# NuTufts/ubresnet

Hardware: AMD Instinct MI355X
Metric: images/sec, 512x512 U-ResNet train step (fwd+loss+bwd+Adam) (higher is better)
Workload: dtype bf16; 1 GPU; ub_uresnet 3-class ip16 bf16, batch 16 per GPU (global 16), 512x512x1 synthetic LArTPC crops, Adam(1e-5, wd 1e-4); parallelism=dp1, global_batch=16, optimizer=ubresnet_amd.optim.FlatAdam

## Files before the change

### ubresnet_amd/csrc/ubr_conv.hip

```cpp
#include <stdlib.h>
#include <type_traits>
#include "ubr_common.h"
#include "ubr_host.h"

namespace {

struct ConvK {
  const char* x; long x_sn, x_sy, x_sx;
  const float *in_sub, *in_scale, *in_shift, *in_lo;
  const char* w;
  char* y; long y_sn, y_sy, y_sx;
  const char* ad; long a_sn, a_sy, a_sx;
  const float* bias;
  double* stats;
  int H, W;
  int CU, UPB, lgUPB, nblk;
  int Cout, Cout_pad;
  int ntaps, S, iy0, ix0, OH, OW;
  int dymin, dxmin, HH, HW;
  int tiles_x, tiles_y;
  unsigned tx_magic, ty_magic;
  int nunits, steps;
  int pixb;
  unsigned rw, rw_magic;
// ... 531 lines not shown
        }
        const int vo = (okp[i] && okc[j]) ? lane_y : kOut;
        if constexpr (sizeof(T) == 2) {
          uint2 pk;
          store4<T>(reinterpret_cast<char*>(&pk), v);
          __builtin_amdgcn_raw_buffer_store_b64(ubr_u2{pk.x, pk.y}, yr, vo, so_y[i] + j * 16 * ESZ, 0);
        } else {
          buf_store16(ubr_u4{__float_as_uint(v[0]), __float_as_uint(v[1]), __float_as_uint(v[2]), __float_as_uint(v[3])}, yr, vo, so_y[i] + j * 16 * ESZ);
        }
      }
    }
  } else
#pragma unroll
  for (int j = 0; j < NT; ++j) {
    const int ch = n0 + j * 16 + 4 * q;
    float4 bmu = make_float4(0.f, 0.f, 0.f, 0.f), bsc = bmu, bsh = bmu, bis = bmu;
    const bool bnb = k.bc != nullptr && ch < k.Cout;
    if (bnb) {
      bmu = *reinterpret_cast<const float4*>(k.bmean + ch); bsc = *reinterpret_cast<const float4*>(k.bscale + ch);
      bsh = *reinterpret_cast<const float4*>(k.bshift + ch); bis = *reinterpret_cast<const float4*>(k.binvstd + ch);
    }
    auto finish = [&](int i, float* v, int& oy, int& ox) -> bool {
      const int f = wave * FW + i;
      oy = oy0 + f / TWF; ox = ox0 + (f % TWF) * 16 + l16;
      const bool valid = (oy < k.OH) && (ox < k.OW);
#pragma unroll
      for (int r = 0; r < 4; ++r) v[r] = acc[i][j][r] + bs[j][r];
      if (k.act & 1) {
#pragma unroll
        for (int r = 0; r < 4; ++r) v[r] = fmaxf(v[r], 0.f);
      }
      if (adb != nullptr && valid && ch < k.Cout) {
        float a4[4];
        load4<T>(adb + (long)n * k.a_sn + (long)oy * k.a_sy + (long)ox * k.a_sx + (long)ch * ESZ, a4);
        if (k.ad_mask != nullptr) {
          const unsigned mb = (unsigned)k.ad_mask[(((long)n * k.OH + oy) * k.OW + ox) * k.ad_mask_cu + ch / CPU] >> (ch % CPU);
#pragma unroll
          for (int r = 0; r < 4; ++r) a4[r] = ((mb >> r) & 1u) ? a4[r] : 0.f;
        }
#pragma unroll
        for (int r = 0; r < 4; ++r) v[r] += a4[r];
      }
      if (k.act & 2) {
#pragma unroll
        for (int r = 0; r < 4; ++r) v[r] = fmaxf(v[r], 0.f);
      }
      if (k.stats != nullptr && valid) {
        if (k.bc != nullptr) {
          if (bnb) {
            float g4[4], c4[4];
            round4<T>(v, g4);
            load4<T>(k.bc + (long)n * k.bc_sn + (long)oy * k.bc_sy + (long)ox * k.bc_sx + (long)ch * ESZ, c4);
            bnb_accumulate(g4, c4, bmu, bsc, bsh, bis, s1[j], s2[j]);
          }
        } else {
#pragma unroll
          for (int r = 0; r < 4; ++r) { s1[j][r] += v[r]; s2[j][r] += v[r] * v[r]; }
        }
      }
      return valid;
    };
    constexpr bool PAIRS = (FW % 2 == 0) && sizeof(T) == 2;
    if (PAIRS && k.pair_store && k.epilogue == 0) {
#pragma unroll
      for (int i = 0; i < FW; i += 2) {
        float v0[4], v1[4];
        int oy_a, ox_a, oy_b, ox_b;
        const bool ok0 = finish(i, v0, oy_a, ox_a) && ch < k.Cout;
        const bool ok1 = finish(i + (FW > 1 ? 1 : 0), v1, oy_b, ox_b) && ch < k.Cout;
        store_frag_pair<T>(yb + (long)n * k.y_sn + (long)oy_a * k.y_sy + (long)ox_a * k.y_sx + (long)ch * ESZ,
                           yb + (long)n * k.y_sn + (long)oy_b * k.y_sy + (long)ox_b * k.y_sx + (long)ch * ESZ, ok0, ok1, v0, v1, q);
      }
    } else {
#pragma unroll
    for (int i = 0; i < FW; ++i) {
      float v[4];
      int oy, ox;
      const bool valid = finish(i, v, oy, ox);
      if (k.epilogue == 0) {
        if (valid && ch < k.Cout)
          store4<T>(yb + (long)n * k.y_sn + (long)oy * k.y_sy + (long)ox * k.y_sx + (long)ch * ESZ, v);
      } else if (j == 0) {
        float m = -3.0e38f;
#pragma unroll
        for (int r = 0; r < 4; ++r) if (ch + r < k.Cout) m = fmaxf(m, v[r]);
        m = fmaxf(m, __shfl_xor(m, 16, 64));
        m = fmaxf(m, __shfl_xor(m, 32, 64));
        float e = 0.f;
#pragma unroll
        for (int r = 0; r < 4; ++r) if (ch + r < k.Cout) e += expf(v[r] - m);
        e += __shfl_xor(e, 16, 64);
        e += __shfl_xor(e, 32, 64);
        const float lse = m + logf(e);
        if (valid) {
          float* o = reinterpret_cast<float*>(k.y);
#pragma unroll
          for (int r = 0; r < 4; ++r)
            if (ch + r < k.Cout) o[(((long)n * k.Cout + ch + r) * k.OH + oy) * k.OW + ox] = v[r] - lse;
        }
      }
    }
    }
  }

#ifdef UBR_CONV_STAMPS
  const unsigned long long te1 = __builtin_amdgcn_s_memtime();
#endif
  if (k.stats != nullptr) {
#pragma unroll
    for (int j = 0; j < NT; ++j)
#pragma unroll
      for (int r = 0; r < 4; ++r) {
        const float a = wave_quadrow_sum16(s1[j][r]);
        const float b = wave_quadrow_sum16(s2[j][r]);
        if (l16 == 0) {
          red[(wave * TN + j * 16 + 4 * q + r) * 2 + 0] = a;
          red[(wave * TN + j * 16 + 4 * q + r) * 2 + 1] = b;
        }
      }
    __syncthreads();
    if (tid < TN) {
      const int ch = n0 + tid;
      if (ch < k.Cout) {
        double a = 0.0, b = 0.0;
#pragma unroll
        for (int w = 0; w < 4; ++w) { a += (double)red[(w * TN + tid) * 2]; b += (double)red[(w * TN + tid) * 2 + 1]; }
        double* st = k.stats + (size_t)(blockIdx.x % k.nslots) * 2 * k.Cout;
        atomicAdd(&st[ch], a);
        atomicAdd(&st[k.Cout + ch], b);
      }
    }
  }
#ifdef UBR_CONV_STAMPS
  if (PIPE && k.stamps != nullptr) {
    const unsigned long long te2 = __builtin_amdgcn_s_memtime();
    __syncthreads();
    if (tid == 0) {
      unsigned long long* o = k.stamps + ((size_t)blockIdx.y * gridDim.x + blockIdx.x) * 16;
      o[9] = __builtin_amdgcn_s_memtime(); o[11] = te0; o[12] = te1; o[13] = te2;
    }
  }
#endif
}

struct ThinK {
  const char* x; long x_sn; int x_sy, x_sx; unsigned x_bytes;
  const float *in_sub, *in_scale, *in_shift, *in_lo;
  const char* w;
  char* y; long y_sn; int y_sy, y_sx; unsigned y_bytes;
  const char* ad; long a_sn; int a_sy, a_sx; unsigned a_bytes;
  const float* bias; double* stats;
  int H, W, HW, nitems; unsigned hw_magic;
  int tiles_x, tiles_y, ntiles; unsigned tx_magic, ty_magic;
  int steps, nunits, hy_org, hx_org, dymin, dxmin;
  int Cout, Cout_pad, CU, OH, OW;
  int act, epilogue, wlinear, dbg;
  int wl_off, halo_off, red_off;
  int8_t dy[UBR_MAX_TAPS], dx[UBR_MAX_TAPS];
  uint8_t wt[UBR_MAX_TAPS];
  unsigned long long* stamps;
  const uint8_t* ad_mask; int ad_mask_cu; unsigned mask_bytes;
  const char* bc; long bc_sn; int bc_sy, bc_sx; unsigned bc_bytes;
  const float *bmean, *bscale, *bshift, *binvstd;
  int nslots;
  int nphase, pstep0[4], psteps[4], pyoff[4];
};


template <typename T, int FW, int NT, int TWF, int UPB, bool XF, bool LSM, bool ROW7 = false, int EXT = 0>
__global__ __launch_bounds__(256, ((ROW7 || (EXT == 1 && NT == 2)) ? 2 : 3)) void conv_thin_kernel(const ThinK k) {
  ubr_main_prio();
  static_assert(EXT == 0 || (!XF && !LSM), "the training epilogues belong to the data-gradient convs (no transform on load, NHWC output)");
  constexpr int TN = NT * 16;
  constexpr int TH = 4 * FW / TWF;
  constexpr int TW = TWF * 16;
  constexpr int CPU = ET<T>::CPU;
  constexpr int ESZ = 16 / CPU;
  constexpr int LG = UPB == 4 ? 2 : (UPB == 2 ? 1 : 0);
  constexpr int PIXB = thin_pixb(UPB);
  constexpr int HS = ROW7 ? 7 : (UPB == 4 ? 6 : 5);
  constexpr int PPS = 256 / UPB;
  constexpr int WB = 4;
  constexpr int FH = ROW7 ? 8 : 4;
  static_assert(TWF == 2 && FW % FH == 0, "tile shape");
  static_assert(!ROW7 || (FW == 8 && NT == 1 && UPB == 2), "ROW7 is the 16x32-pixel, 16-cout, 16-cin tile");
  constexpr bool WIDE = ESZ == 2;

  extern __shared__ __attribute__((aligned(16))) char smem[];
  int* tbl = reinterpret_cast<int*>(smem);
  char* wl = smem + k.wl_off;
  char* halo = smem + k.halo_off;
  float* red = reinterpret_cast<float*>(smem + k.red_off);

  const int tid = threadIdx.x, lane = tid & 63, wave = tid >> 6, q = lane >> 4, l16 = lane & 15;
  const int n0 = blockIdx.y * TN;
  const int c = tid & (UPB - 1);
  const int nw = 4 * k.steps * TN;

  int hxu[HS], relu[HS];
  int hyu[XF ? HS : 1];
#pragma unroll
  for (int u = 0; u < HS; ++u) {
    const int pix = (tid >> LG) + u * PPS;
    const int hy = (int)udiv_magic((unsigned)pix, k.hw_magic), hx = pix - hy * k.HW;
    const bool in = tid + u * 256 < k.nitems;
    hxu[u] = in ? hx : -(1 << 24);
    relu[u] = hy * k.x_sy + hx * k.x_sx + c * 16;
    if constexpr (XF) hyu[u] = hy;
  }
  char* const halo_w = halo + (tid >> LG) * PIXB + c * 16;

  ubr_u4 hv[HS];
  unsigned hok = 0u;
  auto load_halo = [&](int tile) {
    const unsigned t = (unsigned)__builtin_amdgcn_readfirstlane(tile);
    const unsigned r = udiv_magic(t, k.tx_magic), tx = t - r * (unsigned)k.tiles_x;
    const unsigned n = udiv_magic(r, k.ty_magic), ty = r - n * (unsigned)k.tiles_y;
    const int hy0 = (int)ty * TH + k.hy_org, hx0 = (int)tx * TW + k.hx_org;
    __amdgpu_buffer_rsrc_t xr = __builtin_amdgcn_make_buffer_rsrc((void*)(k.x + (long)n * k.x_sn), 0, (int)k.x_bytes, 0x00020000);
    const int goff = hy0 * k.x_sy + hx0 * k.x_sx;
    hok = 0u;
#pragma unroll
    for (int u = 0; u < HS; ++u) {
      const bool ok = (unsigned)(hx0 + hxu[u]) < (unsigned)k.W;
      int vo = ok ? relu[u] + goff : -1;
      if (k.dbg & 1) vo = -1;
      hv[u] = __builtin_amdgcn_raw_buffer_load_b128(xr, vo, 0, 0);
      if constexpr (XF) hok |= (unsigned)(ok & ((unsigned)(hy0 + hyu[u]) < (unsigned)k.H)) << u;
    }
  };

  const int ntiles = k.ntiles;
  int tile = blockIdx.x;
  load_halo(tile);
  uint4 wv[WB];
  if (k.wlinear) {
    const int nvalid = k.nunits * TN;
#pragma unroll
    for (int u = 0; u < WB; ++u) {
      const int i = tid + u * 256;
      wv[u] = make_uint4(0u, 0u, 0u, 0u);
      if (i < nvalid) wv[u] = ldg16(k.w + (long)i * 16);
    }
  }
  float bs[NT][4];
#pragma unroll
  for (int j = 0; j < NT; ++j)
#pragma unroll
    for (int r = 0; r < 4; ++r) {
      const int ch = n0 + j * 16 + 4 * q + r;
      bs[j][r] = (k.bias != nullptr && ch < k.Cout) ? k.bias[ch] : 0.f;
    }
  float* xfc = red + 4 * TN * 2;
  if constexpr (XF) {
    for (int i = tid; i < 4 * UPB * CPU; i += 256) {
      const int which = i / (UPB * CPU), ch = i - which * (UPB * CPU);
      const float* src = which == 0 ? k.in_sub : (which == 1 ? k.in_scale : (which == 2 ? k.in_shift : k.in_lo));
      xfc[i] = src[ch];
    }
  }
  if constexpr (EXT == 1) {
    for (int i = tid; i < 4 * TN; i += 256) {
      const int which = i / TN, ch = n0 + (i - which * TN);
      const float* src = which == 0 ? k.bmean : (which == 1 ? k.bscale : (which == 2 ? k.bshift : k.binvstd));
      xfc[i] = ch < k.Cout ? src[ch] : 0.f;
    }
  }
  int* wsrc = tbl + 4 * k.steps;
  for (int u = tid; u < 4 * k.steps; u += 256) {
    int off = 0, v = -1;
    if (u < k.nunits) {
      const int tap = u >> LG, cc = u & (UPB - 1);
      off = ((k.dy[tap] - k.dymin) * k.HW + (k.dx[tap] - k.dxmin)) * PIXB + cc * 16;
      v = k.wt[tap] == 255 ? -1 : ((int)k.wt[tap] * k.CU + cc) * k.Cout_pad;
    }
    tbl[u] = off;
    wsrc[u] = v;
  }
  if (k.wlinear) {
#pragma unroll
    for (int u = 0; u < WB; ++u) {
      const int i = tid + u * 256;
      if (i < nw) *reinterpret_cast<uint4*>(wl + (long)i * 16) = wv[u];
    }
    const int nvalid = k.nunits * TN;
    for (int ib = tid + 256 * WB; ib < nw; ib += 256 * WB) {
#pragma unroll
      for (int u = 0; u < WB; ++u) {
        const int i = ib + u * 256;
        wv[u] = make_uint4(0u, 0u, 0u, 0u);
        if (i < nvalid) wv[u] = ldg16(k.w + (long)i * 16);
      }
#pragma unroll
      for (int u = 0; u < WB; ++u) {
        const int i = ib + u * 256;
        if (i < nw) *reinterpret_cast<uint4*>(wl + (long)i * 16) = wv[u];
      }
    }
  } else {
    __syncthreads();
    for (int ib = tid; ib < nw; ib += 256 * WB) {
#pragma unroll
      for (int u = 0; u < WB; ++u) {
        const int i = ib + u * 256;
        wv[u] = make_uint4(0u, 0u, 0u, 0u);
        if (i < nw) {
          const int src = wsrc[i / TN];
          if (src >= 0) wv[u] = ldg16(k.w + ((long)(src + n0 + (i % TN))) * 16);
        }
      }
#pragma unroll
      for (int u = 0; u < WB; ++u) {
        const int i = ib + u * 256;
        if (i < nw) *reinterpret_cast<uint4*>(wl + (long)i * 16) = wv[u];
      }
    }
  }

  if constexpr (XF || EXT == 1) __syncthreads();
  const int fb0 = (((wave * FW) / TWF) * k.HW + l16) * PIXB;
  const int rowb = k.HW * PIXB;
  int vo_out[NT];
#pragma unroll
  for (int j = 0; j < NT; ++j) {
    if constexpr (WIDE) vo_out[j] = ((wave * FW) / TWF) * k.y_sy + ((q & 1) * 16 + l16) * k.y_sx + (n0 + j * 16 + 8 * (q >> 1)) * ESZ;
    else vo_out[j] = ((wave * FW) / TWF) * k.y_sy + l16 * k.y_sx + (n0 + j * 16 + 4 * q) * ESZ;
  }
  int vo_ad[NT];
#pragma unroll
  for (int j = 0; j < NT; ++j) vo_ad[j] = ((wave * FW) / TWF) * k.a_sy + l16 * k.a_sx + (n0 + j * 16 + 4 * q) * ESZ;
  int vo_c[EXT == 1 ? NT : 1], vo_m[EXT == 2 ? NT : 1];
  if constexpr (EXT == 1) {
#pragma unroll
    for (int j = 0; j < NT; ++j) vo_c[j] = ((wave * FW) / TWF) * k.bc_sy + l16 * k.bc_sx + (n0 + j * 16 + 4 * q) * ESZ;
  }
  if constexpr (EXT == 2) {
#pragma unroll
    for (int j = 0; j < NT; ++j) vo_m[j] = (((wave * FW) / TWF) * k.OW + l16) * k.ad_mask_cu + (n0 + j * 16 + 4 * q) / CPU;
  }
  float s1[NT][4], s2[NT][4];
#pragma unroll
  for (int j = 0; j < NT; ++j)
#pragma unroll
    for (int r = 0; r < 4; ++r) { s1[j][r] = 0.f; s2[j][r] = 0.f; }

#ifdef UBR_CONV_STAMPS
  unsigned long long tS = 0, tL = 0, tC = 0, tE = 0, tB = 0, tW = 0, t_ = __builtin_amdgcn_s_memtime();
  const unsigned long long t_begin = t_;
#define UBR_TSTAMP(acc_) do { unsigned long long n_ = __builtin_amdgcn_s_memtime(); acc_ += n_ - t_; t_ = n_; } while (0)
#else
#define UBR_TSTAMP(acc_) do { } while (0)
#endif
  while (tile < ntiles) {
#ifdef UBR_CONV_STAMPS
    asm volatile("s_waitcnt vmcnt(0)" ::: "memory");
    UBR_TSTAMP(tW);
#endif
    float xsub[XF ? CPU : 1], xsc[XF ? CPU : 1], xsh[XF ? CPU : 1], xlo[XF ? CPU : 1];
    if constexpr (XF) {
#pragma unroll
      for (int e = 0; e < CPU; ++e) {
        xsub[e] = xfc[0 * UPB * CPU + c * CPU + e]; xsc[e] = xfc[1 * UPB * CPU + c * CPU + e];
        xsh[e] = xfc[2 * UPB * CPU + c * CPU + e]; xlo[e] = xfc[3 * UPB * CPU + c * CPU + e];
      }
    }
#pragma unroll
    for (int u = 0; u < HS; ++u) {
      uint4 v = __builtin_bit_cast(uint4, hv[u]);
      if constexpr (XF) {
        if ((hok >> u) & 1u) {
          float f[CPU];
          ET<T>::unpack(v, f);
          ubr_bnrelu<CPU>(f, xsub, xsc, xsh, xlo);
          v = ET<T>::pack(f);
        }
      }
      if (tid + u * 256 < k.nitems) *reinterpret_cast<uint4*>(halo_w + u * (PPS * PIXB)) = v;
    }
    UBR_TSTAMP(tS);
    __syncthreads();
    UBR_TSTAMP(tB);
    const unsigned t = (unsigned)__builtin_amdgcn_readfirstlane(tile);
    const unsigned rr = udiv_magic(t, k.tx_magic), tx = t - rr * (unsigned)k.tiles_x;
    const unsigned n = udiv_magic(rr, k.ty_magic), ty = rr - n * (unsigned)k.tiles_y;
    const int oy0 = (int)ty * TH, ox0 = (int)tx * TW;
    const int next = tile + gridDim.x;
    if (next < ntiles) load_halo(next);
    __amdgpu_buffer_rsrc_t yr = __builtin_amdgcn_make_buffer_rsrc((void*)(k.y + (long)n * k.y_sn), 0, (int)k.y_bytes, 0x00020000);
    __amdgpu_buffer_rsrc_t ar = __builtin_amdgcn_make_buffer_rsrc((void*)(k.ad != nullptr ? k.ad + (long)n * k.a_sn : k.x), 0, k.ad != nullptr ? (int)k.a_bytes : 0, 0x00020000);
    const int ybase = oy0 * k.y_sy + ox0 * k.y_sx, abase = oy0 * k.a_sy + ox0 * k.a_sx;
    __amdgpu_buffer_rsrc_t cr = yr, mr = yr;
    int cbase = 0, mbase = 0;
    if constexpr (EXT == 1) {
      cr = __builtin_amdgcn_make_buffer_rsrc((void*)(k.bc + (long)n * k.bc_sn), 0, (int)k.bc_bytes, 0x00020000);
      cbase = oy0 * k.bc_sy + ox0 * k.bc_sx;
    }
    if constexpr (EXT == 2) {
      mr = __builtin_amdgcn_make_buffer_rsrc((void*)(k.ad_mask + (long)n * k.mask_bytes), 0, (int)k.mask_bytes, 0x00020000);
      mbase = (oy0 * k.OW + ox0) * k.ad_mask_cu;
    }
    UBR_TSTAMP(tL);

#pragma unroll 1
    for (int g0 = 0; g0 < FW; g0 += FH) {
      ubr_u4 adv4[FH][NT];
      ubr_u2 adv2[FH][NT];
      if (k.ad != nullptr) {
#pragma unroll
        for (int i = 0; i < FH; ++i)
#pragma unroll
          for (int j = 0; j < NT; ++j) {
            const int so = abase + ((g0 + i) / TWF) * k.a_sy;
            if constexpr (WIDE) adv2[i][j] = __builtin_amdgcn_raw_buffer_load_b64(ar, vo_ad[j] + (i % TWF) * 16 * k.a_sx, so, 0);
            else adv4[i][j] = __builtin_amdgcn_raw_buffer_load_b128(ar, vo_ad[j] + (i % TWF) * 16 * k.a_sx, so, 0);
          }
      }
      unsigned admk[EXT == 2 ? FH : 1][EXT == 2 ? NT : 1];
      ubr_u4 cv4[EXT == 1 ? FH : 1][EXT == 1 ? NT : 1];
      ubr_u2 cv2[EXT == 1 ? FH : 1][EXT == 1 ? NT : 1];
      if constexpr (EXT == 2) {
#pragma unroll
        for (int i = 0; i < FH; ++i)
#pragma unroll
          for (int j = 0; j < NT; ++j)
            admk[i][j] = __builtin_amdgcn_raw_buffer_load_b8(mr, vo_m[j] + (i % TWF) * 16 * k.ad_mask_cu, mbase + ((g0 + i) / TWF) * k.OW * k.ad_mask_cu, 0);
      }
      if constexpr (EXT == 1) {
#pragma unroll
        for (int i = 0; i < FH; ++i)
#pragma unroll
          for (int j = 0; j < NT; ++j) {
            const int so = cbase + ((g0 + i) / TWF) * k.bc_sy;
            if constexpr (WIDE) cv2[i][j] = __builtin_amdgcn_raw_buffer_load_b64(cr, vo_c[j] + (i % TWF) * 16 * k.bc_sx, so, 0);
            else cv4[i][j] = __builtin_amdgcn_raw_buffer_load_b128(cr, vo_c[j] + (i % TWF) * 16 * k.bc_sx, so, 0);
          }
      }
      const int nph = (ROW7 || LSM || EXT != 0) ? 1 : k.nphase;
#pragma unroll 1
      for (int ph = 0; ph < nph; ++ph) {
      const int s_lo = nph > 1 ? k.pstep0[ph] : 0;
      const int s_cnt = nph > 1 ? k.psteps[ph] : k.steps;
      const int y_ph = nph > 1 ? k.pyoff[ph] : 0;
      f32x4 acc[FH][NT];
#pragma unroll
      for (int i = 0; i < FH; ++i)
#pragma unroll
        for (int j = 0; j < NT; ++j) acc[i][j] = f32x4{0.f, 0.f, 0.f, 0.f};
      const char* hb = halo + fb0 + (g0 / TWF) * rowb;
      if constexpr (ROW7) {
        constexpr int ROWB = (TW + 6) * PIXB;
#pragma unroll 1
        for (int pp = 0; pp < 4; ++pp) {
          const char* pb = hb + tbl[4 * pp + q];
          const char* pw = wl + ((4 * pp + q) * TN + l16) * 16;
          uint4 w7[7];
#pragma unroll
          for (int dy = 0; dy < 7; ++dy) w7[dy] = *reinterpret_cast<const uint4*>(pw + dy * (16 * TN * 16));
#pragma unroll
          for (int ir = 0; ir < 10; ++ir) {
            const uint4 b0 = *reinterpret_cast<const uint4*>(pb + ir * ROWB);
            const uint4 b1 = *reinterpret_cast<const uint4*>(pb + ir * ROWB + 16 * PIXB);
#pragma unroll
            for (int r = 0; r < 4; ++r) {
              const int dy = ir - r;
              if (dy >= 0 && dy <= 6) {
                acc[2 * r][0] = mma_step<T>(acc[2 * r][0], w7[dy], b0);
                acc[2 * r + 1][0] = mma_step<T>(acc[2 * r + 1][0], w7[dy], b1);
              }
            }
          }
        }
      } else {
      int off_n = tbl[4 * s_lo + q];
      uint4 wf_n[NT];
#pragma unroll
      for (int j = 0; j < NT; ++j) wf_n[j] = *reinterpret_cast<const uint4*>(wl + (((4 * s_lo + q) * TN) + j * 16 + l16) * 16);
      const int nsteps = s_lo + ((k.dbg & 2) ? 1 : s_cnt);
      for (int s = s_lo; s < nsteps; ++s) {
        const char* pa = hb + off_n;
        uint4 wf[NT];
#pragma unroll
        for (int j = 0; j < NT; ++j) wf[j] = wf_n[j];
        if (s + 1 < nsteps) {
          off_n = tbl[4 * (s + 1) + q];
#pragma unroll
          for (int j = 0; j < NT; ++j) wf_n[j] = *reinterpret_cast<const uint4*>(wl + (((4 * (s + 1) + q) * TN) + j * 16 + l16) * 16);
        }
        uint4 a[FH];
        a[0] = *reinterpret_cast<const uint4*>(pa);
        a[1] = *reinterpret_cast<const uint4*>(pa + 16 * PIXB);
        a[2] = *reinterpret_cast<const uint4*>(pa + rowb);
        a[3] = *reinterpret_cast<const uint4*>(pa + rowb + 16 * PIXB);
#pragma unroll
        for (int i = 0; i < FH; ++i)
#pragma unroll
          for (int j = 0; j < NT; ++j) acc[i][j] = mma_step<T>(acc[i][j], wf[j], a[i]);
      }
      }
      UBR_TSTAMP(tC);

#pragma unroll
      for (int i = 0; i < FH; i += 2) {
#pragma unroll
        for (int j = 0; j < NT; ++j) {
          float v[2][4];
#pragma unroll
          for (int h = 0; h < 2; ++h) {
#pragma unroll
            for (int r = 0; r < 4; ++r) v[h][r] = acc[i + h][j][r] + bs[j][r];
            if (k.act & 1) {
#pragma unroll
              for (int r = 0; r < 4; ++r) v[h][r] = fmaxf(v[h][r], 0.f);
            }
            if (k.ad != nullptr) {
              float a4[4];
              if constexpr (WIDE) {
                const uint2 raw = make_uint2(adv2[i + h][j][0], adv2[i + h][j][1]);
                load4<T>(reinterpret_cast<const char*>(&raw), a4);
              } else {
                const uint4 raw = __builtin_bit_cast(uint4, adv4[i + h][j]);
                ET<T>::unpack(raw, a4);
              }
              if constexpr (EXT == 2) {
                const unsigned mb = (admk[i + h][j] & 0xffu) >> ((n0 + j * 16 + 4 * q) % CPU);
#pragma unroll
                for (int r = 0; r < 4; ++r) v[h][r] = __builtin_fmaf(a4[r], (float)((mb >> r) & 1u), v[h][r]);
              } else {
#pragma unroll
                for (int r = 0; r < 4; ++r) v[h][r] += a4[r];
              }
            }
            if (k.act & 2) {
#pragma unroll
              for (int r = 0; r < 4; ++r) v[h][r] = fmaxf(v[h][r], 0.f);
            }
            if constexpr (EXT == 1) {
              float g4[4], c4[4];
              round4<T>(v[h], g4);
              if constexpr (WIDE) {
                const uint2 raw = make_uint2(cv2[i + h][j][0], cv2[i + h][j][1]);
                load4<T>(reinterpret_cast<const char*>(&raw), c4);
              } else {
                const uint4 raw = __builtin_bit_cast(uint4, cv4[i + h][j]);
                ET<T>::unpack(raw, c4);
              }
              const float* cc = xfc + j * 16 + 4 * q;
              bnb_accumulate(g4, c4, *reinterpret_cast<const float4*>(cc), *reinterpret_cast<const float4*>(cc + TN),
                             *reinterpret_cast<const float4*>(cc + 2 * TN), *reinterpret_cast<const float4*>(cc + 3 * TN), s1[j], s2[j]);
            } else if (k.stats != nullptr) {
#pragma unroll
              for (int r = 0; r < 4; ++r) { s1[j][r] += v[h][r]; s2[j][r] += v[h][r] * v[h][r]; }
            }
          }
          const int so = ybase + ((g0 + i) / TWF) * k.y_sy + y_ph;
          if constexpr (!LSM) {
            if (k.dbg & 4) {
              if (v[0][0] == 1.2345e-30f && v[1][1] == 1.2345e-30f) __builtin_amdgcn_raw_buffer_store_b32(__float_as_uint(v[0][0]), yr, vo_out[j], so, 0);
            } else if constexpr (WIDE) {
              const uint4 pk = pack_swap_pair<T>(v[0], v[1]);
              ubr_u4 o = {pk.x, pk.y, pk.z, pk.w};
              buf_store16(o, yr, vo_out[j], so);
            } else {
#pragma unroll
              for (int h = 0; h < 2; ++h) {
                ubr_u4 o = {__float_as_uint(v[h][0]), __float_as_uint(v[h][1]), __float_as_uint(v[h][2]), __float_as_uint(v[h][3])};
                buf_store16(o, yr, vo_out[j] + h * 16 * k.y_sx, so);
              }
            }
          } else if (j == 0) {
            (void)so;
#pragma unroll
            for (int h = 0; h < 2; ++h) {
              const int ch = 4 * q;
              const int f = wave * FW + g0 + i + h;
              const int oy = oy0 + f / TWF, ox = ox0 + (f % TWF) * 16 + l16;
              float m = -3.0e38f;
#pragma unroll
              for (int r = 0; r < 4; ++r) if (ch + r < k.Cout) m = fmaxf(m, v[h][r]);
              m = fmaxf(m, __shfl_xor(m, 16, 64));
              m = fmaxf(m, __shfl_xor(m, 32, 64));
              float e = 0.f;
#pragma unroll
              for (int r = 0; r < 4; ++r) if (ch + r < k.Cout) e += expf(v[h][r] - m);
              e += __shfl_xor(e, 16, 64);
              e += __shfl_xor(e, 32, 64);
              const float lse = m + logf(e);
              float* o = reinterpret_cast<float*>(k.y);
#pragma unroll
              for (int r = 0; r < 4; ++r)
                if (ch + r < k.Cout) o[(((long)n * k.Cout + ch + r) * k.OH + oy) * k.OW + ox] = v[h][r] - lse;
            }
          }
        }
      }
      }
      UBR_TSTAMP(tE);
    }
    tile = next;
    if (tile < ntiles) __syncthreads();
    UBR_TSTAMP(tB);
  }
#ifdef UBR_CONV_STAMPS
  if (k.stamps != nullptr && tid == 0) {
    unsigned long long* o = k.stamps + ((size_t)blockIdx.y * gridDim.x + blockIdx.x) * 16;
    o[0] = tS; o[1] = tL; o[2] = tC; o[3] = tB; o[6] = tW; o[10] = tE; o[4] = t_ - t_begin; o[5] = t_begin; o[7] = t_begin; o[8] = t_; o[9] = t_;
  }
#endif

  if (k.stats != nullptr) {
#pragma unroll
    for (int j = 0; j < NT; ++j)
#pragma unroll
      for (int r = 0; r < 4; ++r) {
        const float a = wave_quadrow_sum16(s1[j][r]);
        const float b = wave_quadrow_sum16(s2[j][r]);
        if (l16 == 0) {
          red[(wave * TN + j * 16 + 4 * q + r) * 2 + 0] = a;
          red[(wave * TN + j * 16 + 4 * q + r) * 2 + 1] = b;
        }
      }
    __syncthreads();
    if (tid < TN) {
      const int ch = n0 + tid;
      if (ch < k.Cout) {
        double a = 0.0, b = 0.0;
#pragma unroll
        for (int w = 0; w < 4; ++w) { a += (double)red[(w * TN + tid) * 2]; b += (double)red[(w * TN + tid) * 2 + 1]; }
        double* st = k.stats + (size_t)(blockIdx.x % k.nslots) * 2 * k.Cout;
        atomicAdd(&st[ch], a);
        atomicAdd(&st[k.Cout + ch], b);
      }
    }
  }
}

template <typename T, int FW, int TWF, int STEPS>
__global__ __launch_bounds__(512) void conv_pc_kernel(const ConvK k) {
  constexpr int NT = 4, TN = 64;
  constexpr int F = 4 * FW;
  constexpr int TH = F / TWF;
  constexpr int TW = TWF * 16;
  constexpr int CPU = ET<T>::CPU;
  constexpr int ESZ = 16 / CPU;
  constexpr int HS = conv_pipe_hslots(FW, TWF), WS = conv_pipe_wslots(NT);
  constexpr int kOOR = (int)0x80000000;
  static_assert(F % TWF == 0, "tile shape");

  extern __shared__ __attribute__((aligned(16))) char smem[];
  int* tbl = reinterpret_cast<int*>(smem);
  int* wsrc = tbl + 4 * k.steps;
  float* xfc = reinterpret_cast<float*>(smem + k.xfc_off);

  const int tid = threadIdx.x, lane = tid & 63, wave = tid >> 6, q = lane >> 4, l16 = lane & 15;
  const bool producer = wave >= 4;
  const int ptid = tid & 255;
  const bool has_xf = k.in_scale != nullptr;

  for (int u = tid; u < 4 * k.steps; u += 512) {
    int off = 0, v = -1;
    if (u < k.nunits) {
      const int tap = u >> 2, cc = u & 3;
      off = ((k.dy[tap] - k.dymin) * k.HW + (k.dx[tap] - k.dxmin)) * k.pixb + cc * 16;
      v = ((int)k.wt[tap] * k.CU + cc) * k.Cout_pad;
    }
    tbl[u] = off;
    wsrc[u] = v;
  }
  if (has_xf) {
    for (int ch = tid; ch < k.CU * CPU; ch += 512) {
      float* o = xfc + (ch / CPU) * 4 * CPU + (ch % CPU);
      o[0] = k.in_sub[ch]; o[CPU] = k.in_scale[ch]; o[2 * CPU] = k.in_shift[ch]; o[3 * CPU] = k.in_lo[ch];
    }
  }
  __syncthreads();

  const int ntiles = k.tiles_x * k.tiles_y * k.N;
  const int total = ntiles * k.ncot;
  const int G = (int)gridDim.x;
  const int nmine = (int)blockIdx.x < total ? (total - (int)blockIdx.x + G - 1) / G : 0;
  const int niter = nmine * k.nblk;

  float s1[NT][4], s2[NT][4];
#pragma unroll
  for (int j = 0; j < NT; ++j)
#pragma unroll
    for (int r = 0; r < 4; ++r) { s1[j][r] = 0.f; s2[j][r] = 0.f; }

  if (producer) {
    const int c = ptid & 3;
    const int nit = k.HH * (int)k.rw;
    const int nw = 4 * k.steps * TN;
    int h_rc[HS], h_rel[HS];
#pragma unroll
    for (int u = 0; u < HS; ++u) {
      const int it = ptid + u * 256;
      const int hy = (int)__umulhi((unsigned)it, k.rw_magic);
      const int hx = (it - hy * (int)k.rw) >> 2;
      h_rc[u] = it < nit ? ((hy << 16) | hx) : -1;
      h_rel[u] = hy * k.x_sy32 + hx * k.x_sx32 + c * 16;
    }
    int w_rel[WS];
#pragma unroll
    for (int u = 0; u < WS; ++u) {
      const int i = ptid + u * 256;
      int v = kOOR;
      if (i < nw) {
        const int src = wsrc[i / TN];
        if (src >= 0) v = (src + (i % TN)) * 16;
      }
      w_rel[u] = v;
    }
    const __amdgpu_buffer_rsrc_t wr = __builtin_amdgcn_make_buffer_rsrc((void*)k.w, 0, 0x7fffffff, 0x00020000);
    const int x_img = k.H * k.x_sy32;
    const int hfull = nit >> 8, hrem = nit & 255, wfull = nw >> 8, wrem = nw & 255;
    const int halo_inc = 64 * k.pixb;
    char* const halo_w0 = smem + k.halo_off + (ptid >> 2) * k.pixb + c * 16;
    char* const wl_w0 = smem + k.wl_off + ptid * 16;

    int lu = (int)blockIdx.x, lblk = 0;
    int hoff[HS], woff[WS];
    unsigned hok_unit = 0u;
    __amdgpu_buffer_rsrc_t xr = wr;
    auto issue = [&](ubr_u4 (&hv)[HS], ubr_u4 (&wv)[WS], unsigned& hokm) {
      if (lblk == 0) {
        const int u_ = __builtin_amdgcn_readfirstlane(lu);
        const int ct = u_ / ntiles;
        int t = u_ - ct * ntiles;
        const int tx = t % k.tiles_x; t /= k.tiles_x;
        const int ty = t % k.tiles_y;
        const int n = t / k.tiles_y;
        const int hy0 = ty * TH + k.iy0 + k.dymin, hx0 = tx * TW + k.ix0 + k.dxmin;
        xr = __builtin_amdgcn_make_buffer_rsrc((void*)(k.x + (long)n * k.x_sn), 0, x_img, 0x00020000);
        const int org = hy0 * k.x_sy32 + hx0 * k.x_sx32;
        hok_unit = 0u;
#pragma unroll
        for (int u = 0; u < HS; ++u) {
          const int hy = h_rc[u] >> 16, hx = h_rc[u] & 0xffff;
          const bool okx = h_rc[u] >= 0 && (unsigned)(hx0 + hx) < (unsigned)k.W;
          hoff[u] = okx ? h_rel[u] + org : kOOR;
          hok_unit |= (okx && (unsigned)(hy0 + hy) < (unsigned)k.H) ? (1u << u) : 0u;
        }
        const int n0b = ct * TN * 16;
#pragma unroll
        for (int u = 0; u < WS; ++u) woff[u] = w_rel[u] == kOOR ? kOOR : w_rel[u] + n0b;
      }
      const int sh = lblk * 64, sw = lblk * 4 * k.Cout_pad * 16;
#pragma unroll
      for (int u = 0; u < HS; ++u) hv[u] = __builtin_amdgcn_raw_buffer_load_b128(xr, hoff[u], sh, 0);
#pragma unroll
      for (int u = 0; u < WS; ++u) wv[u] = __builtin_amdgcn_raw_buffer_load_b128(wr, woff[u], sw, 0);
      hokm = hok_unit;
      if (++lblk == k.nblk) { lblk = 0; lu += G; }
// ... 329 lines not shown
      unsigned long long* o = k.stamps + (size_t)blockIdx.x * 16;
      o[0] = tC; o[1] = tE; o[2] = tB; o[3] = t_ - t_begin; o[4] = (unsigned long long)niter;
    }
#endif
  }
}

static thread_local int g_last_conv_cfg[4] = {0, 0, 0, 0};
static thread_local char g_last_conv_name[160] = "";
struct TileCfg { int FW, NT, TWF; };
static const TileCfg kCfgs[] = {
    {8, 1, 2},
    {4, 1, 2},
    {4, 2, 2},
    {4, 4, 2},
    {2, 4, 1},
    {1, 4, 1},
    {2, 2, 1},
    {2, 1, 1},
    {1, 2, 1},
    {1, 1, 1},
};
constexpr int kNumCfgs = sizeof(kCfgs) / sizeof(kCfgs[0]);

template <typename T, int FW, int NT, int TWF, bool PIPE>
int launch_one(const ConvK& k, dim3 grid, size_t lds, hipStream_t st) {
  auto fn = conv_igemm_kernel<T, FW, NT, TWF, PIPE>;
  if (lds > 64 * 1024) {
    static thread_local size_t maxset = 0;
    if (lds > maxset) {
      hipError_t e = hipFuncSetAttribute(reinterpret_cast<const void*>(fn), hipFuncAttributeMaxDynamicSharedMemorySize, (int)lds);
      if (e != hipSuccess) { ubr_set_error("ubr_conv: cannot raise LDS limit to %zu: %s", lds, hipGetErrorString(e)); return UBR_ELAUNCH; }
      maxset = lds;
    }
  }
  ubr_launch(fn, grid, dim3(256), lds, st, k);
  UBR_LAUNCH_CHECK("ubr_conv");
  return UBR_OK;
}

template <typename T, int FW, int NT, int TWF, int UPB, bool XF, bool LSM = false, bool ROW7 = false, int EXT = 0>
int launch_thin(const ThinK& k, dim3 grid, size_t lds, hipStream_t st) {
  auto fn = conv_thin_kernel<T, FW, NT, TWF, UPB, XF, LSM, ROW7, EXT>;
  if (lds > 64 * 1024) {
    static thread_local size_t maxset = 0;
    if (lds > maxset) {
      hipError_t e = hipFuncSetAttribute(reinterpret_cast<const void*>(fn), hipFuncAttributeMaxDynamicSharedMemorySize, (int)lds);
      if (e != hipSuccess) { ubr_set_error("ubr_conv: cannot raise LDS limit to %zu: %s", lds, hipGetErrorString(e)); return UBR_ELAUNCH; }
      maxset = lds;
    }
  }
  ubr_launch(fn, grid, dim3(256), lds, st, k);
  UBR_LAUNCH_CHECK("ubr_conv");
  return UBR_OK;
}

static unsigned magic_u32(unsigned d) { return d <= 1 ? 0u : (unsigned)((0x100000000ull + d - 1) / d); }

template <typename T, int FW, int NT, int TWF>
int try_thin(const ConvK& c, dim3 grid, hipStream_t st, int* rc) {
  constexpr int TH = 4 * FW / TWF, TW = TWF * 16, TN = NT * 16;
  static const bool thin_on = [] { const char* e = getenv("UBR_CONV_THIN"); return !e || atoi(e) != 0; }();
  const int esz = 16 / ET<T>::CPU;
  if (!thin_on || c.nblk != 1 || c.S != 1 || (c.UPB != 2 && c.UPB != 4)) return 0;
  const int nph = (int)grid.z;
  int steps_tot = c.steps, nunits_tot = c.nunits;
  if (nph > 1) {
    if (nph > 4 || c.ad != nullptr || c.stats != nullptr || c.epilogue != 0 || c.bc != nullptr || c.ad_mask != nullptr) return 0;
    steps_tot = 0; nunits_tot = 0;
    for (int p = 0; p < nph; ++p) {
      if (c.pnunits[p] % 4 || c.ptap0[p] * c.UPB != nunits_tot || c.pyoff[p] < 0 || c.pyoff[p] >= (1L << 30)) return 0;
      steps_tot += c.psteps[p]; nunits_tot += c.pnunits[p];
    }
    if (nunits_tot != c.ntaps * c.UPB) return 0;
  }
  int map7[7][7];
  bool row7 = false;
  if constexpr (FW == 8 && NT == 1 && sizeof(T) == 2) {
    static const bool row7_on = [] { const char* e = getenv("UBR_CONV_ROW7"); return !e || atoi(e) != 0; }();
    row7 = row7_on && c.ntaps == 49 && c.UPB == 2 && c.dymin == -3 && c.dxmin == -3 && c.HW == TW + 6 && c.HH == TH + 6;
    if (row7) {
      for (int a = 0; a < 7; ++a) for (int b = 0; b < 7; ++b) map7[a][b] = -1;
      for (int t = 0; t < 49 && row7; ++t) {
        const int a = c.dy[t] + 3, b = c.dx[t] + 3;
        if (a < 0 || a > 6 || b < 0 || b > 6 || map7[a][b] >= 0 || c.wt[t] == 255) row7 = false; else map7[a][b] = c.wt[t];
      }
    }
  }
  const int HSn = row7 ? 7 : (c.UPB == 4 ? 6 : 5);
  if (c.HH * (int)c.rw > 256 * HSn) return 0;
  if (c.OH % TH || c.OW % TW) return 0;
  if (c.epilogue == 0 && esz == 2 && !c.wide_store) return 0;
  if (c.epilogue == 0 && (c.Cout % 4 || c.Cout_pad != (int)grid.y * TN)) return 0;
  if (c.x_sy >= (1L << 24) || c.y_sy >= (1L << 24) || (long)c.H * c.x_sy >= (1L << 31) || (long)c.OH * c.y_sy >= (1L << 31)) return 0;
  if (c.ad != nullptr && (c.a_sy >= (1L << 24) || (long)c.OH * c.a_sy >= (1L << 31))) return 0;
  const int ntiles = c.tiles_x * c.tiles_y * c.N;
  if ((unsigned long long)ntiles * (unsigned)c.tiles_x >= (1ull << 32)) return 0;
  ThinK k{};
  k.x = c.x; k.x_sn = c.x_sn; k.x_sy = (int)c.x_sy; k.x_sx = (int)c.x_sx; k.x_bytes = (unsigned)((long)c.H * c.x_sy);
  k.in_sub = c.in_sub; k.in_scale = c.in_scale; k.in_shift = c.in_shift; k.in_lo = c.in_lo;
  k.w = c.w;
  k.y = c.y; k.y_sn = c.y_sn; k.y_sy = (int)c.y_sy; k.y_sx = (int)c.y_sx; k.y_bytes = (unsigned)((long)c.OH * c.y_sy);
  k.ad = c.ad; k.a_sn = c.a_sn; k.a_sy = (int)c.a_sy; k.a_sx = (int)c.a_sx; k.a_bytes = c.ad ? (unsigned)((long)c.OH * c.a_sy) : 0u;
  k.bias = c.bias; k.stats = c.stats;
  k.H = c.H; k.W = c.W; k.HW = c.HW; k.nitems = c.HH * (int)c.rw; k.hw_magic = magic_u32((unsigned)c.HW);
  k.tiles_x = c.tiles_x; k.tiles_y = c.tiles_y; k.ntiles = ntiles;
  k.tx_magic = magic_u32((unsigned)c.tiles_x); k.ty_magic = magic_u32((unsigned)c.tiles_y);
  k.steps = steps_tot; k.nunits = nunits_tot; k.hy_org = c.iy0 + c.dymin; k.hx_org = c.ix0 + c.dxmin; k.dymin = c.dymin; k.dxmin = c.dxmin;
  k.nphase = nph;
  for (int p = 0, s0 = 0; p < 4; ++p) {
    k.pstep0[p] = s0; k.psteps[p] = p < nph ? c.psteps[p] : 0; k.pyoff[p] = p < nph ? (int)c.pyoff[p] : 0;
    s0 += k.psteps[p];
  }
  k.Cout = c.Cout; k.Cout_pad = c.Cout_pad; k.CU = c.CU; k.OH = c.OH; k.OW = c.OW;
  k.act = c.act; k.epilogue = c.epilogue; k.wlinear = nph > 1 ? 0 : c.wlinear; k.dbg = c.dbg; k.stamps = c.stamps;
  for (int t = 0; t < c.ntaps; ++t) { k.dy[t] = c.dy[t]; k.dx[t] = c.dx[t]; k.wt[t] = c.wt[t]; }
  const int ext = c.bc != nullptr ? 1 : (c.ad_mask != nullptr ? 2 : 0);
  if (ext != 0 && (c.in_scale != nullptr || c.epilogue != 0)) return 0;
  k.nslots = c.nslots;
  if (ext == 1) {
    if (c.bc_sy >= (1L << 24) || (long)c.OH * c.bc_sy >= (1L << 31)) return 0;
    k.bc = c.bc; k.bc_sn = c.bc_sn; k.bc_sy = (int)c.bc_sy; k.bc_sx = (int)c.bc_sx; k.bc_bytes = (unsigned)((long)c.OH * c.bc_sy);
    k.bmean = c.bmean; k.bscale = c.bscale; k.bshift = c.bshift; k.binvstd = c.binvstd;
  }
  if (ext == 2) {
    if ((long)c.OH * c.OW * c.ad_mask_cu >= (1L << 31)) return 0;
    k.ad_mask = c.ad_mask; k.ad_mask_cu = c.ad_mask_cu; k.mask_bytes = (unsigned)((long)c.OH * c.OW * c.ad_mask_cu);
  }
  if (row7) {
    for (int a = 0; a < 7; ++a)
      for (int b = 0; b < 8; ++b) {
        const int t = a * 8 + b;
        k.dy[t] = (int8_t)(a - 3); k.dx[t] = (int8_t)((b < 7 ? b : 6) - 3); k.wt[t] = (uint8_t)(b < 7 ? map7[a][b] : 255);
      }
    k.nunits = 56 * 2; k.steps = 28; k.wlinear = 0;
  }
  const int pixb = thin_pixb(c.UPB);
  size_t off = ((size_t)2 * 16 * k.steps + 15) & ~(size_t)15;
  k.wl_off = (int)off; off += (size_t)4 * k.steps * TN * 16;
  k.halo_off = (int)off; off += ((size_t)c.HH * c.HW * pixb + 15) & ~(size_t)15;
  k.red_off = (int)off; off += (size_t)4 * TN * 2 * sizeof(float) + (size_t)4 * 4 * 8 * sizeof(float);
  const size_t lds = off;
  if (lds > 150 * 1024) return 0;
  const size_t lds_budget = 159 * 1024;
  static const int wg_per_cu = [] { const char* e = getenv("UBR_CONV_THIN_WGS"); return e ? atoi(e) : 0; }();
  int per_cu = (int)(lds_budget / lds);
  const int reg_cap = (row7 || (ext == 1 && NT == 2)) ? 2 : (NT == 1 ? (ext == 1 ? 3 : 4) : 3);
  if (per_cu > reg_cap) per_cu = reg_cap;
  if (wg_per_cu > 0) per_cu = wg_per_cu;
  if (per_cu < 1) per_cu = 1;
  dim3 g(grid.x, grid.y);
  const unsigned cap = 256u * (unsigned)per_cu / (grid.y ? grid.y : 1);
  if (g.x > cap && cap > 0) g.x = cap;
  g_last_conv_cfg[3] = 2;
  const bool xf = c.in_scale != nullptr;
  snprintf(g_last_conv_name, sizeof(g_last_conv_name), "conv_thin_kernel<%s, %d, %d, %d, %d, %s, %s, false, 0>", sizeof(T) == 4 ? "float" : (std::is_same<T, bf16_t>::value ? "bf16_t" : "f16_t"),
           FW, NT, TWF, c.UPB, xf ? "true" : "false", c.epilogue == 1 ? "true" : "false");
  if (ext != 0)
    snprintf(g_last_conv_name, sizeof(g_last_conv_name), "conv_thin_kernel<%s, %d, %d, %d, %d, false, false, %s, %d>", sizeof(T) == 4 ? "float" : (std::is_same<T, bf16_t>::value ? "bf16_t" : "f16_t"),
             FW, NT, TWF, c.UPB, row7 ? "true" : "false", ext);
  if constexpr (FW == 8 && NT == 1 && sizeof(T) == 2) {
    if (row7) {
      if (ext == 0)
      snprintf(g_last_conv_name, sizeof(g_last_conv_name), "conv_thin_kernel<%s, 8, 1, 2, 2, %s, %s, true, 0>", std::is_same<T, bf16_t>::value ? "bf16_t" : "f16_t",
               xf ? "true" : "false", c.epilogue == 1 ? "true" : "false");
      if (c.epilogue == 1) *rc = xf ? launch_thin<T, 8, 1, 2, 2, true, true, true>(k, g, lds, st) : launch_thin<T, 8, 1, 2, 2, false, true, true>(k, g, lds, st);
      else if (ext == 1) *rc = launch_thin<T, 8, 1, 2, 2, false, false, true, 1>(k, g, lds, st);
      else if (ext == 2) *rc = launch_thin<T, 8, 1, 2, 2, false, false, true, 2>(k, g, lds, st);
      else *rc = xf ? launch_thin<T, 8, 1, 2, 2, true, false, true>(k, g, lds, st) : launch_thin<T, 8, 1, 2, 2, false, false, true>(k, g, lds, st);
      return 1;
    }
  }
  if (c.epilogue == 1) {
    if constexpr (FW == 4 && NT == 1) {
      if (c.UPB != 2) return 0;
      *rc = xf ? launch_thin<T, FW, NT, TWF, 2, true, true>(k, g, lds, st) : launch_thin<T, FW, NT, TWF, 2, false, true>(k, g, lds, st);
      return 1;
    } else {
      return 0;
    }
  }
  if (ext == 1) *rc = c.UPB == 2 ? launch_thin<T, FW, NT, TWF, 2, false, false, false, 1>(k, g, lds, st) : launch_thin<T, FW, NT, TWF, 4, false, false, false, 1>(k, g, lds, st);
  else if (ext == 2) *rc = c.UPB == 2 ? launch_thin<T, FW, NT, TWF, 2, false, false, false, 2>(k, g, lds, st) : launch_thin<T, FW, NT, TWF, 4, false, false, false, 2>(k, g, lds, st);
  else if (c.UPB == 2) *rc = xf ? launch_thin<T, FW, NT, TWF, 2, true>(k, g, lds, st) : launch_thin<T, FW, NT, TWF, 2, false>(k, g, lds, st);
  else *rc = xf ? launch_thin<T, FW, NT, TWF, 4, true>(k, g, lds, st) : launch_thin<T, FW, NT, TWF, 4, false>(k, g, lds, st);
  return 1;
}

template <typename T, int FW, int NT, int TWF>
int launch_cfg(const ConvK& k, dim3 grid, size_t lds, hipStream_t st) {
  if constexpr (NT <= 2 && TWF == 2) {
    int rc = UBR_OK;
    if (try_thin<T, FW, NT, TWF>(k, grid, st, &rc)) return rc;
  }
  if constexpr (NT == 4) {
    static const bool enabled = [] { const char* e = getenv("UBR_CONV_PIPE"); return !e || atoi(e) != 0; }();
    if (enabled && k.nblk >= 2 && k.HH * (int)k.rw <= 256 * conv_pipe_hslots(FW, TWF) && 4 * k.steps * NT * 16 <= 256 * conv_pipe_wslots(NT))
      { g_last_conv_cfg[3] = 1; return launch_one<T, FW, NT, TWF, true>(k, grid, lds, st); }
  }
  g_last_conv_cfg[3] = 0;
  return launch_one<T, FW, NT, TWF, false>(k, grid, lds, st);
}

template <typename T, int FW, int TWF, int STEPS>
int launch_pc_steps(const ConvK& k, dim3 grid, size_t lds, hipStream_t st) {
  auto fn = conv_pc_kernel<T, FW, TWF, STEPS>;
  if (lds > 64 * 1024) {
    static thread_local size_t maxset = 0;
    if (lds > maxset) {
      hipError_t e = hipFuncSetAttribute(reinterpret_cast<const void*>(fn), hipFuncAttributeMaxDynamicSharedMemorySize, (int)lds);
      if (e != hipSuccess) { ubr_set_error("ubr_conv: cannot raise LDS limit to %zu: %s", lds, hipGetErrorString(e)); return UBR_ELAUNCH; }
      maxset = lds;
    }
  }
  ubr_launch(fn, grid, dim3(512), lds, st, k);
  UBR_LAUNCH_CHECK("ubr_conv");
  return UBR_OK;
}

template <typename T, int FW, int TWF>
int launch_pc_one(const ConvK& k, dim3 grid, size_t lds, hipStream_t st) {
  if (k.steps == 9) return launch_pc_steps<T, FW, TWF, 9>(k, grid, lds, st);
  if (k.steps == 4) return launch_pc_steps<T, FW, TWF, 4>(k, grid, lds, st);
  return launch_pc_steps<T, FW, TWF, 0>(k, grid, lds, st);
}

template <typename T>
int launch_pc(int pi, const ConvK& k, dim3 grid, size_t lds, hipStream_t st) {
  g_last_conv_cfg[3] = 3;
  switch (pi) {
    case 0: return launch_pc_one<T, 4, 2>(k, grid, lds, st);
    case 1: return launch_pc_one<T, 2, 2>(k, grid, lds, st);
    case 2: return launch_pc_one<T, 4, 1>(k, grid, lds, st);
    case 3: return launch_pc_one<T, 2, 1>(k, grid, lds, st);
  }
  ubr_set_error("ubr_conv: bad producer/consumer tile %d", pi);
  return UBR_EINVAL;
}

template <typename T>
int launch_T(int cfg, const ConvK& k, dim3 grid, size_t lds, hipStream_t st) {
  if (cfg >= 100) return launch_pc<T>(cfg - 100, k, grid, lds, st);
  switch (cfg) {
    case 0: return launch_cfg<T, 8, 1, 2>(k, grid, lds, st);
    case 1: return launch_cfg<T, 4, 1, 2>(k, grid, lds, st);
    case 2: return launch_cfg<T, 4, 2, 2>(k, grid, lds, st);
    case 3: return launch_cfg<T, 4, 4, 2>(k, grid, lds, st);
    case 4: return launch_cfg<T, 2, 4, 1>(k, grid, lds, st);
    case 5: return launch_cfg<T, 1, 4, 1>(k, grid, lds, st);
    case 6: return launch_cfg<T, 2, 2, 1>(k, grid, lds, st);
    case 7: return launch_cfg<T, 2, 1, 1>(k, grid, lds, st);
    case 8: return launch_cfg<T, 1, 2, 1>(k, grid, lds, st);
    case 9: return launch_cfg<T, 1, 1, 1>(k, grid, lds, st);
  }
  ubr_set_error("ubr_conv: bad tile config %d", cfg);
  return UBR_EINVAL;
}

struct Plan { int cfg; size_t lds; int UPB, steps, HH, HW, pixb, wl_off, halo_off, red_off, xfc_off, tiles_x, tiles_y, pc_buf; };

static int eff_ntaps(const ubr_conv_desc* d) {
  if (d->nphase <= 1) return d->ntaps;
  int m = 0;
  for (int p = 0; p < d->nphase && p < 4; ++p) m = d->phase_ntaps[p] > m ? d->phase_ntaps[p] : m;
  return m;
}

static bool plan_tile(const ubr_conv_desc* d, int cfg, int TH, int TW, int TN, int dymin, int dymax, int dxmin, int dxmax, Plan* p) {
  if (d->Cout_pad % TN) return false;
  if (d->epilogue == 1 && TN != 16) return false;
  const int cpu = ubr_cpu(d->dtype);
  const int CU = d->Cin / cpu;
  int UPB = (CU % 4 == 0) ? 4 : (CU % 2 == 0 ? 2 : 1);
  if (UPB == 4 && (d->S == 2 || eff_ntaps(d) >= 16)) UPB = 2;
  const int nunits = eff_ntaps(d) * UPB;
  const int steps = (nunits + 3) / 4;
  const int HH = (TH - 1) * d->S + 1 + (dymax - dymin);
  const int HW = (TW - 1) * d->S + 1 + (dxmax - dxmin);
  const int pixb = conv_pixb(UPB);
  size_t off = ((size_t)2 * 16 * steps + 15) & ~(size_t)15;
  p->wl_off = (int)off; off += (size_t)4 * steps * TN * 16;
  p->halo_off = (int)off; off += (size_t)HH * HW * pixb;
  off = (off + 15) & ~(size_t)15;
  p->red_off = (int)off; off += (size_t)4 * TN * 2 * sizeof(float);
  p->xfc_off = (int)off;
  if (d->xf.scale != nullptr && CU / UPB >= 2) off += (size_t)d->Cin * 4 * sizeof(float);
  p->cfg = cfg; p->lds = off; p->UPB = UPB; p->steps = steps; p->HH = HH; p->HW = HW; p->pixb = pixb;
  p->tiles_x = ubr_cdiv(d->OW, TW); p->tiles_y = ubr_cdiv(d->OH, TH);
  if ((size_t)HH * HW * UPB >= 60000) return false;
  return off <= 160 * 1024;
}

static bool plan_for(const ubr_conv_desc* d, int cfg, int dymin, int dymax, int dxmin, int dxmax, Plan* p) {
  const TileCfg& c = kCfgs[cfg];
  return plan_tile(d, cfg, 4 * c.FW / c.TWF, c.TWF * 16, c.NT * 16, dymin, dymax, dxmin, dxmax, p);
}

struct PcCfg { int FW, TWF; };
static const PcCfg kPc[] = {
    {4, 2},
    {2, 2},
    {4, 1},
    {2, 1},
};
constexpr int kNumPc = sizeof(kPc) / sizeof(kPc[0]);

// ... 451 lines not shown
```

Before: 1398 images/sec.

## Walk thin-conv tiles in vertical runs and reuse overlapping halo rows in LDS

Replaces the flat grid-stride tile loop in the thin conv kernel with column runs: each block walks a segment of vertically adjacent tiles. It keeps the halo rows that overlap the next tile in LDS, copying them down instead of reloading them from global memory. The host picks a segment length that balances rounds against run length and caps the grid at the run count. This is meant to cut redundant halo loads. In exchange it adds an LDS copy done by one wave, more index logic, and possibly worse load balance across blocks.

New measurement: 1311 images/sec. 6.2% lower.

```diff
diff --git a/ubresnet_amd/csrc/ubr_conv.hip b/ubresnet_amd/csrc/ubr_conv.hip
--- a/ubresnet_amd/csrc/ubr_conv.hip
+++ b/ubresnet_amd/csrc/ubr_conv.hip
@@ -707,6 +707,7 @@
   const float* bias; double* stats;
   int H, W, HW, nitems; unsigned hw_magic;
   int tiles_x, tiles_y, ntiles; unsigned tx_magic, ty_magic;
+  int nruns, segs, seg_len, keep, rw; unsigned seg_magic;
   int steps, nunits, hy_org, hx_org, dymin, dxmin;
   int Cout, Cout_pad, CU, OH, OW;
   int act, epilogue, wlinear, dbg;
@@ -765,29 +766,54 @@
   }
   char* const halo_w = halo + (tid >> LG) * PIXB + c * 16;
 
+  const int rowb = k.HW * PIXB;
+
+  auto decode = [&](int run, int& n, int& tx, int& ty, int& ty_end) {
+    const unsigned r = (unsigned)__builtin_amdgcn_readfirstlane(run);
+    if constexpr (ROW7) {
+      const unsigned rr = udiv_magic(r, k.tx_magic), nn = udiv_magic(rr, k.ty_magic);
+      tx = (int)(r - rr * (unsigned)k.tiles_x); n = (int)nn; ty = (int)(rr - nn * (unsigned)k.tiles_y); ty_end = ty + 1;
+    } else {
+      const unsigned col = udiv_magic(r, k.seg_magic), sg = r - col * (unsigned)k.segs, nn = udiv_magic(col, k.tx_magic);
+      n = (int)nn; tx = (int)(col - nn * (unsigned)k.tiles_x); ty = (int)sg * k.seg_len;
+      ty_end = ty + k.seg_len < k.tiles_y ? ty + k.seg_len : k.tiles_y;
+    }
+  };
   ubr_u4 hv[HS];
   unsigned hok = 0u;
-  auto load_halo = [&](int tile) {
-    const unsigned t = (unsigned)__builtin_amdgcn_readfirstlane(tile);
-    const unsigned r = udiv_magic(t, k.tx_magic), tx = t - r * (unsigned)k.tiles_x;
-    const unsigned n = udiv_magic(r, k.ty_magic), ty = r - n * (unsigned)k.tiles_y;
-    const int hy0 = (int)ty * TH + k.hy_org, hx0 = (int)tx * TW + k.hx_org;
+  auto load_halo = [&](int n, int tx, int ty, int kp) {
+    const int hy0 = ty * TH + k.hy_org + kp, hx0 = tx * TW + k.hx_org;
+    const int lim = k.nitems - kp * k.rw;
     __amdgpu_buffer_rsrc_t xr = __builtin_amdgcn_make_buffer_rsrc((void*)(k.x + (long)n * k.x_sn), 0, (int)k.x_bytes, 0x00020000);
     const int goff = hy0 * k.x_sy + hx0 * k.x_sx;
     hok = 0u;
 #pragma unroll
     for (int u = 0; u < HS; ++u) {
-      const bool ok = (unsigned)(hx0 + hxu[u]) < (unsigned)k.W;
-      int vo = ok ? relu[u] + goff : -1;
-      if (k.dbg & 1) vo = -1;
-      hv[u] = __builtin_amdgcn_raw_buffer_load_b128(xr, vo, 0, 0);
-      if constexpr (XF) hok |= (unsigned)(ok & ((unsigned)(hy0 + hyu[u]) < (unsigned)k.H)) << u;
+      if (u * 256 < lim) {
+        const bool ok = ((unsigned)(hx0 + hxu[u]) < (unsigned)k.W) & (tid + u * 256 < lim);
+        int vo = ok ? relu[u] + goff : -1;
+        if (k.dbg & 1) vo = -1;
+        hv[u] = __builtin_amdgcn_raw_buffer_load_b128(xr, vo, 0, 0);
+        if constexpr (XF) hok |= (unsigned)(ok & ((unsigned)(hy0 + hyu[u]) < (unsigned)k.H)) << u;
+      }
     }
   };
 
-  const int ntiles = k.ntiles;
-  int tile = blockIdx.x;
-  load_halo(tile);
+  auto step = [&](int run, int ty, int& nrun, int& nty, int& nkeep) {
+    int n_, tx_, t0, te;
+    decode(run, n_, tx_, t0, te);
+    nrun = run; nty = ty + 1; nkeep = k.keep;
+    if (nty >= te) {
+      nrun = run + (int)gridDim.x; nkeep = 0; nty = 0;
+      if (nrun < k.nruns) { decode(nrun, n_, tx_, t0, te); nty = t0; }
+    }
+  };
+  int run = blockIdx.x, ty = 0;
+  if (run < k.nruns) {
+    int n_, tx_, te;
+    decode(run, n_, tx_, ty, te);
+    load_halo(n_, tx_, ty, 0);
+  }
   uint4 wv[WB];
   if (k.wlinear) {
     const int nvalid = k.nunits * TN;
@@ -874,7 +900,6 @@
 
   if constexpr (XF || EXT == 1) __syncthreads();
   const int fb0 = (((wave * FW) / TWF) * k.HW + l16) * PIXB;
-  const int rowb = k.HW * PIXB;
   int vo_out[NT];
 #pragma unroll
   for (int j = 0; j < NT; ++j) {
@@ -906,7 +931,10 @@
 #else
 #define UBR_TSTAMP(acc_) do { } while (0)
 #endif
-  while (tile < ntiles) {
+  while (run < k.nruns) {
+    int n, tx, ty_first, ty_end;
+    decode(run, n, tx, ty_first, ty_end);
+    const int hkeep = ty > ty_first ? k.keep : 0;
 #ifdef UBR_CONV_STAMPS
     asm volatile("s_waitcnt vmcnt(0)" ::: "memory");
     UBR_TSTAMP(tW);
@@ -930,17 +958,21 @@
           v = ET<T>::pack(f);
         }
       }
-      if (tid + u * 256 < k.nitems) *reinterpret_cast<uint4*>(halo_w + u * (PPS * PIXB)) = v;
+      if (tid + u * 256 < k.nitems - hkeep * k.rw) *reinterpret_cast<uint4*>(halo_w + hkeep * rowb + u * (PPS * PIXB)) = v;
     }
     UBR_TSTAMP(tS);
     __syncthreads();
     UBR_TSTAMP(tB);
-    const unsigned t = (unsigned)__builtin_amdgcn_readfirstlane(tile);
-    const unsigned rr = udiv_magic(t, k.tx_magic), tx = t - rr * (unsigned)k.tiles_x;
-    const unsigned n = udiv_magic(rr, k.ty_magic), ty = rr - n * (unsigned)k.tiles_y;
-    const int oy0 = (int)ty * TH, ox0 = (int)tx * TW;
-    const int next = tile + gridDim.x;
-    if (next < ntiles) load_halo(next);
+    const int oy0 = ty * TH, ox0 = tx * TW;
+    {
+      int nrun, nty, nkeep;
+      step(run, ty, nrun, nty, nkeep);
+      if (nrun < k.nruns) {
+        int nn, ntx, t0, te;
+        decode(nrun, nn, ntx, t0, te);
+        load_halo(nn, ntx, nty, nkeep);
+      }
+    }
     __amdgpu_buffer_rsrc_t yr = __builtin_amdgcn_make_buffer_rsrc((void*)(k.y + (long)n * k.y_sn), 0, (int)k.y_bytes, 0x00020000);
     __amdgpu_buffer_rsrc_t ar = __builtin_amdgcn_make_buffer_rsrc((void*)(k.ad != nullptr ? k.ad + (long)n * k.a_sn : k.x), 0, k.ad != nullptr ? (int)k.a_bytes : 0, 0x00020000);
     const int ybase = oy0 * k.y_sy + ox0 * k.y_sx, abase = oy0 * k.a_sy + ox0 * k.a_sx;
@@ -1151,8 +1183,25 @@
       }
       UBR_TSTAMP(tE);
     }
-    tile = next;
-    if (tile < ntiles) __syncthreads();
+    int nrun, nty, nkeep;
+    asm volatile("" : "+s"(run), "+s"(ty));
+    step(run, ty, nrun, nty, nkeep);
+    if constexpr (!ROW7) {
+      if (wave == 0 && nkeep > 0) {
+        const int cnt = nkeep * k.rw;
+        char* dst = halo + (lane >> LG) * PIXB + (lane & (UPB - 1)) * 16;
+        for (int i0 = 0; i0 < cnt; i0 += 128, dst += (128 >> LG) * PIXB) {
+          const bool ok0 = i0 + lane < cnt, ok1 = i0 + 64 + lane < cnt;
+          uint4 c0 = make_uint4(0u, 0u, 0u, 0u), c1 = c0;
+          if (ok0) c0 = *reinterpret_cast<const uint4*>(dst + TH * rowb);
+          if (ok1) c1 = *reinterpret_cast<const uint4*>(dst + TH * rowb + (64 >> LG) * PIXB);
+          if (ok0) *reinterpret_cast<uint4*>(dst) = c0;
+          if (ok1) *reinterpret_cast<uint4*>(dst + (64 >> LG) * PIXB) = c1;
+        }
+      }
+    }
+    run = nrun; ty = nty;
+    if (run < k.nruns) __syncthreads();
     UBR_TSTAMP(tB);
   }
 #ifdef UBR_CONV_STAMPS
@@ -1788,6 +1837,21 @@
   dim3 g(grid.x, grid.y);
   const unsigned cap = 256u * (unsigned)per_cu / (grid.y ? grid.y : 1);
   if (g.x > cap && cap > 0) g.x = cap;
+  k.rw = (int)c.rw;
+  k.keep = (!row7 && c.HH - TH >= 0 && c.HH - TH <= FW / TWF) ? c.HH - TH : 0;
+  k.seg_len = 1;
+  if (!row7) {
+    const long cols = (long)c.tiles_x * c.N;
+    long best = -1;
+    for (int L = 1; L <= c.tiles_y; ++L) {
+      const long segs = (c.tiles_y + L - 1) / L, rounds = (cols * segs + g.x - 1) / g.x;
+      if (best < 0 || rounds * L <= best) { best = rounds * L; k.seg_len = L; }
+    }
+  }
+  k.segs = row7 ? 1 : (c.tiles_y + k.seg_len - 1) / k.seg_len;
+  k.nruns = row7 ? ntiles : c.tiles_x * c.N * k.segs;
+  k.seg_magic = magic_u32((unsigned)k.segs);
+  if (g.x > (unsigned)k.nruns) g.x = (unsigned)k.nruns;
   g_last_conv_cfg[3] = 2;
   const bool xf = c.in_scale != nullptr;
   snprintf(g_last_conv_name, sizeof(g_last_conv_name), "conv_thin_kernel<%s, %d, %d, %d, %d, %s, %s, false, 0>", sizeof(T) == 4 ? "float" : (std::is_same<T, bf16_t>::value ? "bf16_t" : "f16_t"),
```
